# safijari/yag-slam

Measured on AMD Instinct MI355X. Metric: pose hypotheses/sec, higher is better.
Workload: dtype u8

## Files before the change

yag_slam_amd/csrc/ym_host_enqueue.hpp:

```cpp
void enqueue_prepare(ym_matcher *m, const CallPlan &P) {
    ym::PrepareArgs a;
    a.scans = P.d_scans; a.items = P.d_items; a.g = P.g; a.lat = P.lc; a.states = m->states.p; a.qlocal = m->qlocal.p;
    a.cells = m->cells.p; a.bbox = m->bbox.p; a.ctrig = m->ctrig.p; a.hypcell = m->hypcell.p; a.probs = P.probs;
    a.max_n = P.max_n; a.max_base = P.max_base; a.nt_stride = P.nt_stride; a.dim_stride = P.dim_stride; a.stamps = P.stamps;
    a.use_inline = P.inline_desc ? 1 : 0;
    a.pad0 = 0;
    std::memset(&a.inl, 0, sizeof a.inl);
    if (a.use_inline) {
        a.inl.item = P.hi[0];
        for (int i = 0; i < P.nscans; i++) a.inl.scans[i] = P.hs[i];
    }
    a.qnp = m->qnp.p; a.jobs = P.d_jobs; a.job_slot = P.d_job_slot;
    a.fault = nullptr; a.step = 0; a.pad1 = 0;
    for (int k = 0; k < 4; k++) a.cell_box[k] = P.cell_box[k];
    if (P.chain_step) { a.fault = m->seq_fault.p; a.step = P.chain_step; }
    a.tile_max_zero = P.use_tile_list ? m->tile_max.p : nullptr;
    const size_t lds = YM_PREP_LDS_BYTES(P.max_n);
    if (P.split_prepare) {
        if (P.n_jobs > 0) hipLaunchKernelGGL(ym::points_kernel, dim3(P.n_jobs), dim3(YM_POINTS_THREADS), lds, m->stream, a);
        hipLaunchKernelGGL(ym::cells_kernel, dim3(P.max_base + 1, P.B), dim3(256), 0, m->stream, a);
    } else {
        if (P.B == 1 && m->prepare_threads != 512)
            hipLaunchKernelGGL(ym::prepare_kernel<1024>, dim3(P.max_base + 2, P.B), dim3(1024), lds, m->stream, a);
        else
            hipLaunchKernelGGL(ym::prepare_kernel<512>, dim3(P.max_base + 2, P.B), dim3(512), lds, m->stream, a);
    }
}

int enqueue_select(ym_matcher *m, const CallPlan &P) {
    if (P.g.zone_count <= 1) return YM_OK;
    const size_t pts = (size_t)P.max_base * P.max_n;
    int log2cap = 10;
    while (((size_t)3 << log2cap) < 4 * pts) log2cap++;
    if (log2cap > 17 || P.g.storage_w >= 32768)
        return set_err(YM_ERR_UNSUPPORTED, "order-dependent smear (smear_deviation/resolution = %g): chains of more than 98304 readings are not supported",
                       m->cfg.smear_deviation / m->cfg.resolution);
    if (log2cap > 14 || m->select_global) {
        const size_t cap = (size_t)1 << log2cap;
        const int nb = 5;
        int rc = m->sel_scratch.ensure((size_t)P.B * cap * (3 + (nb - 1)));
        if (rc) return rc;
        ym::SelectGlobalArgs g;
        g.cells = m->cells.p; g.max_n = P.max_n; g.max_base = P.max_base; g.z2max = m->z2max; g.log2cap = log2cap;
        g.keys = m->sel_scratch.p; g.status = g.keys + (size_t)P.B * cap; g.minidx = g.status + (size_t)P.B * cap; g.nbr = g.minidx + (size_t)P.B * cap;
        HIP_TRY(hipMemsetAsync(g.keys, 0, (size_t)2 * P.B * cap * sizeof(unsigned), m->stream));
        HIP_TRY(hipMemsetAsync(g.minidx, 0xff, (size_t)P.B * cap * sizeof(unsigned), m->stream));
        const size_t lds = cap;
        hipLaunchKernelGGL(ym::select_global_kernel<5>, dim3(P.B), dim3(1024), lds, m->stream, g);
        return YM_OK;
    }
    if (m->z2max <= 1 && P.B <= m->select_split_max) {
        const size_t cap = (size_t)1 << log2cap;
        const size_t had = m->sel_tables.cap;
        int rc = m->sel_tables.ensure((size_t)2 * P.B * cap);
        if (rc) return rc;
        if (m->sel_tables.cap != had) HIP_TRY(hipMemsetAsync(m->sel_tables.p, 0, m->sel_tables.cap * sizeof(unsigned), m->stream));
        if ((rc = m->sel_rec.ensure((size_t)P.B * 12 * 1024))) return rc;
        if ((rc = m->sel_slot.ensure((size_t)P.B * pts))) return rc;
        ym::SelectSplitArgs s;
        s.cells = m->cells.p; s.max_n = P.max_n; s.max_base = P.max_base; s.log2cap = log2cap; s.pad = 0;
        s.keys = m->sel_tables.p; s.mx = s.keys + (size_t)P.B * cap; s.rec = m->sel_rec.p; s.slot_of = m->sel_slot.p; s.stamps = P.stamps;
        const dim3 grid((unsigned)((pts + YM_SELECT_SPLIT_THREADS - 1) / YM_SELECT_SPLIT_THREADS), P.B);
        hipLaunchKernelGGL(ym::select_hash_kernel, grid, dim3(YM_SELECT_SPLIT_THREADS), 0, m->stream, s);
        hipLaunchKernelGGL(ym::select_neighbours_kernel, grid, dim3(YM_SELECT_SPLIT_THREADS), 0, m->stream, s);
        hipLaunchKernelGGL(ym::select_relax_kernel, dim3(P.B), dim3(1024), cap, m->stream, s);
        return YM_OK;
    }
    ym::SelectArgs a;
    a.cells = m->cells.p; a.max_n = P.max_n; a.max_base = P.max_base; a.z2max = m->z2max; a.log2cap = log2cap; a.stamps = P.stamps;
    const size_t lds = (size_t)9 << log2cap;
    hipLaunchKernelGGL(ym::select_kernel<5>, dim3(P.B), dim3(1024), lds, m->stream, a);
    return YM_OK;
}

int enqueue_raster(ym_matcher *m, const CallPlan &P) {
    hipStream_t st = m->stream;
    const YmGeom &g = P.g;
    if (P.use_tile_list) {
        ym::TilesArgs t;
        t.bbox = m->bbox.p; t.tile_list = m->tile_list.p; t.tile_count = m->tile_count.p; t.tile_zero = m->tile_zero.p;
        t.tile_max = m->tile_max.p;
        t.hits = P.use_tile_hits ? m->tile_hits.p : nullptr; t.tile_h = P.tile_h;
        t.hit_limit = m->raster_hits_per_tile > 0 ? std::min(m->raster_hits_per_tile, YM_TILE_HITS) : YM_TILE_HITS;
        t.max_n = P.max_n; t.max_base = P.max_base; t.half_kernel = g.half_kernel;
        t.tiles_x = P.tiles_x; t.tiles_y = P.tiles_y; t.tile_cap = P.tile_cap;
        for (int k = 0; k < 4; k++) t.launch[k] = P.launch[k];
        hipLaunchKernelGGL(ym::tiles_kernel, dim3(P.B), dim3(YM_TILES_THREADS),
                           (size_t)4 * ((P.tiles_x * P.tiles_y + 31) / 32) + (P.use_tile_hits ? (size_t)8 * P.tile_cap : 0), st, t);
    }
    ym::RasterArgs a;
    a.tiles_x = P.tiles_x; a.tiles_y = P.tiles_y; a.tile_x0 = P.launch[0]; a.tile_y0 = P.launch[1]; a.ltx = P.ltx;
    a.tile_list = P.use_tile_list ? m->tile_list.p : nullptr; a.tile_count = m->tile_count.p; a.tile_cap = P.tile_cap;
    a.cells = m->cells.p; a.bbox = m->bbox.p; a.states = m->states.p; a.g = g; a.grid = m->grid.p;
    a.grid_stride = P.grid_stride; a.planes = m->planes.p; a.lut = m->ktab.p; a.max_n = P.max_n; a.max_base = P.max_base; a.stamps = P.stamps;
    a.tile_zero = m->tile_zero.p; a.sub_zero = m->sub_zero.p; a.planes_only = m->raster_planes_only;
    a.n_rowtab = m->raster_no_rowtab ? 0 : m->n_rowtab; a.rowtab = reinterpret_cast<const uint2 *>(m->rowtab.p); a.rowtab_shift = m->rowtab_shift; a.no_planes = P.win_only ? 1 : 0;
    const size_t rlds = YM_RASTER_LDS_BYTES(P.tile_h, g.half_kernel, a.n_rowtab);
    a.tile_max = m->tile_max.p; a.tile_max_host = P.use_tile_list ? reinterpret_cast<int32_t *>(m->tile_max_host.p) : nullptr;
    a.hits = (P.use_tile_list && P.use_tile_hits) ? m->tile_hits.p : nullptr; a.lty = P.lty; a.pad0 = 0;
    int rc;
    hipEvent_t ev_k = nullptr;
    if ((rc = prof_begin(m, 1, &ev_k))) return rc;
    if (P.ltx > 0 && P.lty > 0) {
        const int hint = m->tile_max_host.p ? *reinterpret_cast<volatile int32_t *>(m->tile_max_host.p) : 0;
        const int gx = m->raster_gx > 0 ? std::min(P.ltx * P.lty, m->raster_gx)
                                        : hint > 0 ? std::min(P.ltx * P.lty, hint + hint / 8 + 2) : P.ltx * P.lty;
        a.first_overflow = gx;
        if (P.use_tile_list) {
            if (P.tile_h == YM_TILE_H_TALL) {
                hipLaunchKernelGGL((ym::raster_kernel<128, false, YM_TILE_H_TALL, true>), dim3(gx, P.B), dim3(128), rlds, st, a);
                if (gx < P.ltx * P.lty) hipLaunchKernelGGL((ym::raster_kernel<128, true, YM_TILE_H_TALL, true>), dim3(4, P.B), dim3(128), rlds, st, a);
            } else {
                hipLaunchKernelGGL((ym::raster_kernel<128, false, YM_TILE_H, true>), dim3(gx, P.B), dim3(128), rlds, st, a);
                if (gx < P.ltx * P.lty) hipLaunchKernelGGL((ym::raster_kernel<128, true, YM_TILE_H, true>), dim3(4, P.B), dim3(128), rlds, st, a);
            }
        } else {
            if (P.tile_h == YM_TILE_H_TALL) hipLaunchKernelGGL((ym::raster_kernel<256, false, YM_TILE_H_TALL, false>), dim3(P.ltx * P.lty, P.B), dim3(256), rlds, st, a);
            else hipLaunchKernelGGL((ym::raster_kernel<256, false, YM_TILE_H, false>), dim3(P.ltx * P.lty, P.B), dim3(256), rlds, st, a);
        }
    }
    return prof_end(m, ev_k);
}

int enqueue_correlate(ym_matcher *m, const CallPlan &P);
void enqueue_score(ym_matcher *m, Slot &slot, const CallPlan &P);

int enqueue_yagpy_passes(ym_matcher *m, Slot &slot, const CallPlan &P) {
    const Call &call = slot.call;
    const YmGeom &g = P.g;
    m->sums_pass_offset[0] = 0;
    m->sums_pass_offset[1] = (size_t)P.B * P.yvol;
    for (int pass = 0; pass < (call.refine ? 2 : 1); pass++) {
        ym::YagArgs a;
        std::memset(&a, 0, sizeof a);
        a.g = g; a.pass = pass; a.penalize = call.penalize; a.refine = call.refine;
        a.last = (pass == 1 || !call.refine) ? 1 : 0;
        if (pass == 0) {
            a.search_xy = m->cfg.search_size * 0.5; a.step_xy = g.res * 2;
            a.search_t = m->cfg.coarse_search_angle_offset * 0.5; a.step_t = m->cfg.coarse_angle_resolution;
        } else {
            a.search_xy = g.res * 2; a.step_xy = g.res; a.search_t = 0.0349 * 0.5; a.step_t = 0.00349;
        }
        a.coarse_angle_res = m->cfg.coarse_angle_resolution;
        a.states = m->states.p; a.host_out = reinterpret_cast<YmItemState *>(slot.result.dp);
        a.qlocal = m->qlocal.p; a.axes = m->yaxes.p; a.rot = nullptr;
        a.sums = m->sums.p + m->sums_pass_offset[pass]; a.out = m->resp.p;
        a.grid = m->grid.p; a.grid_stride = P.grid_stride; a.vol_stride = P.yvol;
        a.max_n = P.max_n; a.maxd = P.ymaxd; a.maxt = P.ymaxt;
        hipLaunchKernelGGL(ym::yag_setup_kernel, dim3(1, P.B), dim3(256), 0, m->stream, a);
        if (pass == 0 && P.lc.nx > 0) {
            a.lat_nx = P.lc.nx; a.lat_ny = P.lc.ny; a.lat_nt = P.lc.nt; a.step_cells = P.sx;
            a.nt_stride = P.nt_stride; a.dim_stride = P.dim_stride; a.ctrig = m->ctrig.p; a.hypcell = m->hypcell.p;
            a.lsums = m->sums.p + (size_t)2 * P.B * P.yvol; a.lsums_stride = P.sums_c; a.counters = m->yag_counters.p;
            hipLaunchKernelGGL(ym::yag_lattice_kernel, dim3(P.B), dim3(256), 0, m->stream, a);
            int rc = enqueue_correlate(m, P);
            if (rc) return rc;
            enqueue_score(m, slot, P);
        }
        if (pass == 1 && m->yag_fast) {
            a.fine_rows = m->yag_fast;
            a.n_items = P.B;
            if (P.B >= 64) hipLaunchKernelGGL(ym::yag_fine_kernel<64>, dim3(8 * P.ymaxt * ((P.B + 7) / 8)), dim3(64), 0, m->stream, a);
            else hipLaunchKernelGGL(ym::yag_fine_kernel<256>, dim3(8 * P.ymaxt * ((P.B + 7) / 8)), dim3(256), 0, m->stream, a);
        }
        hipLaunchKernelGGL(ym::yag_score_kernel, dim3((P.ymaxd * P.ymaxd + 255) / 256, P.ymaxt, P.B), dim3(256), 0, m->stream, a);
        if (P.B >= 16) hipLaunchKernelGGL(ym::yag_reduce_kernel<256>, dim3(P.B), dim3(256), 0, m->stream, a);
        else hipLaunchKernelGGL(ym::yag_reduce_kernel<1024>, dim3(P.B), dim3(1024), 0, m->stream, a);
    }
    return YM_OK;
}

ym::RegionArgs region_args(ym_matcher *m, const CallPlan &P) {
    ym::RegionArgs r;
// ... 212 lines not shown
```

yag_slam_amd/csrc/ym_k_prepare.hpp:

```cpp
#pragma once

namespace ym {

#define YM_PREP_LDS_BYTES(max_n) ((size_t)(max_n) * 25 + ((size_t)(max_n) / 64 + 2) * 4 + 16)
#define YM_INLINE_SCANS 16
#ifndef YM_CELLS_Q
#define YM_CELLS_Q 3
#endif
struct YmInlineDesc {
    YmItem item;
    YmScanRef scans[YM_INLINE_SCANS];
};
struct PrepareArgs {
    const YmScanRef *scans;
    const YmItem *items;
    int32_t use_inline;
    int32_t pad0;
    YmInlineDesc inl;
    YmGeom g;
    YmLattice lat;
    YmItemState *states;
    double2 *qlocal;
    int32_t *qnp;
    YmCell *cells;
    int4 *bbox;
    double2 *ctrig;
    int32_t *hypcell;
    double *probs;
    int32_t max_n, max_base, nt_stride, dim_stride;
    const int32_t *jobs;
    const int32_t *job_slot;
    unsigned long long *stamps;
    int32_t *fault;
    int32_t step, pad1;
    int32_t cell_box[4];
    int32_t *tile_max_zero;
};

struct PrepLds {
    double *sx, *sy;
    int *nxt, *ex, *ent;
    unsigned char *chain;
};
__device__ __forceinline__ PrepLds prep_lds(unsigned char *raw, int max_n) {
    PrepLds l;
    l.sx = reinterpret_cast<double *>(raw);
    l.sy = l.sx + max_n;
    l.nxt = reinterpret_cast<int *>(l.sy + max_n);
    l.ex = l.nxt + max_n;
    l.ent = l.ex + max_n;
    l.chain = reinterpret_cast<unsigned char *>(l.ent + max_n / 64 + 2);
    return l;
}

template <int NT>
__device__ __forceinline__ int project_points(const YmScanRef &sr, double px, double py, double pt, bool yag, double *sx, double *sy,
                                              int *s_cnt , int32_t *cidx_out = nullptr) {
    constexpr int NW = NT / 64;
    const int tid = threadIdx.x;
    const int lane_ = tid & 63, wave_ = tid >> 6;
    const int per = (sr.n + NT - 1) / NT;
    auto valid = [&](int i, double &r) {
        r = 0.0;
        if (i >= sr.n) return false;
        r = sr.ranges[i];
        return yag ? !(r > sr.range_threshold || isnan(r)) : (r >= sr.min_range && r <= sr.range_threshold);
    };
    for (int k = 0; k < per; k++) {
        double r;
        const unsigned long long m = __ballot(valid(k * NT + tid, r));
        if (lane_ == 0) s_cnt[k * NW + wave_] = __popcll(m);
    }
    __syncthreads();
    int running = 0;
    for (int k = 0; k < per; k++) {
        const int i = k * NT + tid;
        double r;
        const bool ok = valid(i, r);
        const unsigned long long m = __ballot(ok);
        int before = 0, total = 0;
#pragma unroll
        for (int w = 0; w < NW; w++) {
            const int c = s_cnt[k * NW + w];
            before += w < wave_ ? c : 0;
            total += c;
        }
        const int pos = running + before + __popcll(m & ((1ull << lane_) - 1ull));
        if (ok) {
            const double angle = pt + sr.min_angle + i * sr.angle_inc;
            sx[pos] = px + r * cos(angle);
            sy[pos] = py + r * sin(angle);
        }
        if (cidx_out && i < sr.n) cidx_out[i] = ok ? pos : -1;
        running += total;
    }
    __syncthreads();
    return running;
}

template <int NT>
__device__ __forceinline__ int project_points_indexed(const YmScanRef &sr, double px, double py, double pt, const PrepLds &l, bool with_gov) {
    for (int i = threadIdx.x; i < sr.n; i += NT) {
        const int pos = sr.cidx[i];
        const double r = sr.ranges[i];
        if (pos >= 0) {
            const double angle = pt + sr.min_angle + i * sr.angle_inc;
            l.sx[pos] = px + r * cos(angle);
            l.sy[pos] = py + r * sin(angle);
        }
    }
    if (with_gov) {
        const int2 *gov = reinterpret_cast<const int2 *>(sr.gov);
        for (int i = threadIdx.x; i < sr.cnp; i += NT) {
            const int2 g = gov[i];
            l.nxt[i] = g.x;
            l.ex[i] = g.y;
        }
    }
    __syncthreads();
    return sr.cnp;
}

#define YM_CHAIN_GUARD 1e-9
#define YM_CHAIN_POSE_LIMIT 1.0e4
#define YM_CHAIN_HEADING_LIMIT 1.0e3
template <int NT, bool GUARD = false>
__device__ __forceinline__ int mark_chain(const PrepLds &l, int np, bool yag) {
    const int tid = threadIdx.x;
    const double min_sq = yag ? 0.2 * 0.2 : 0.1 * 0.1;
    int near = 0;
    for (int i = tid; i < np; i += NT) {
        const double fx = l.sx[i], fy = l.sy[i];
        int j = i + 1;
        for (; j < np; j++) {
            const double dx = fx - l.sx[j], dy = fy - l.sy[j];
            const double d2 = dx * dx + dy * dy;
            if (GUARD) near |= fabs(d2 - min_sq) <= YM_CHAIN_GUARD ? 1 : 0;
            if (d2 > min_sq) break;
        }
        l.nxt[i] = j;
        l.chain[i] = 0;
    }
    int unsafe = 0;
    if (GUARD) unsafe = __syncthreads_or(near);
    else __syncthreads();
    constexpr int SEG = 64;
    const int nseg = (np + SEG - 1) / SEG;
    for (int i = tid; i < np; i += NT) {
        const int seg_end = min(np, (i / SEG + 1) * SEG);
        int j = l.nxt[i];
        while (j < seg_end) j = l.nxt[j];
        l.ex[i] = j;
    }
    for (int i = tid; i < nseg; i += NT) l.ent[i] = -1;
    __syncthreads();
    if (tid == 0)
        for (int cur = 0; cur < np; cur = l.ex[cur]) l.ent[cur / SEG] = cur;
    __syncthreads();
    for (int sgi = tid; sgi < nseg; sgi += NT) {
        int c = l.ent[sgi];
        if (c >= 0) {
// ... 60 lines not shown
    if (tid < a.lat.nt) {
        const double angle = (sr.pose[2] - a.lat.angle_off) + tid * a.lat.angle_res;
        a.ctrig[(size_t)b * a.nt_stride + tid] = make_double2(cos(angle), sin(angle));
    }
    for (int i = tid; i < a.lat.nx * a.lat.ny; i += NT) a.probs[(size_t)b * a.lat.nx * a.lat.ny + i] = 0.0;
    int32_t *cx = a.hypcell + (size_t)b * 2 * a.dim_stride;
    int32_t *cy = cx + a.dim_stride;
    for (int i = tid; i < a.lat.nx; i += NT) cx[i] = hyp_cell(sr.pose[0], -a.lat.off_x, i, a.lat.step_x, off_x, a.g);
    for (int i = tid; i < a.lat.ny; i += NT) cy[i] = hyp_cell(sr.pose[1], -a.lat.off_y, i, a.lat.step_y, off_y, a.g);
    __syncthreads();
    {
        const int stx = kt_round_int(a.lat.step_x * a.g.scale), sty = kt_round_int(a.lat.step_y * a.g.scale);
        int ok = a.g.kpitch == 0;
        for (int i = tid; i < a.lat.nx; i += NT) ok &= (cx[i] == cx[0] + i * stx);
        for (int i = tid; i < a.lat.ny; i += NT) ok &= (cy[i] == cy[0] + i * sty);
        ok = __syncthreads_and(ok);
        if (tid == 0) a.states[b].regular[0] = ok;
    }
}

__device__ __forceinline__ void chain_check_cell(const PrepareArgs &a, int2 c) {
    if (a.fault && c.x != YM_CELL_NONE && (c.x < a.cell_box[0] || c.y < a.cell_box[1] || c.x > a.cell_box[2] || c.y > a.cell_box[3]))
        atomicCAS(a.fault, 0, a.step);
}

template <int NT, typename PT, typename GOV>
__device__ __forceinline__ void prepare_cells(const PrepareArgs &a, int b, int slot, int np, bool yag, double vpx, double vpy,
                                              double off_x, double off_y, PT pt_of, GOV gov_of) {
    const int tid = threadIdx.x;
    const int n_cchunks = YM_N_BOXES(a.max_n);
    YmCell *cells = a.cells + ((size_t)b * a.max_base + slot) * a.max_n;
    int4 *bbox = a.bbox + ((size_t)b * a.max_base + slot) * n_cchunks;
    for (int i0 = 0; i0 < n_cchunks * YM_BOX_CELLS; i0 += NT) {
        const int i = i0 + tid;
        int2 c = make_int2(YM_CELL_NONE, YM_CELL_NONE);
        if (i < np) {
            bool keep = false;
            const int2 g = gov_of(i);
            if (g.x >= 0 && g.y < np) {
                const double2 f = pt_of(g.x), cp = pt_of(g.y);
                const double fx = f.x, fy = f.y, cx = cp.x, cy = cp.y;
                const double aa = vpy - fy;
                const double bb = fx - vpx;
                const double cc = fy * vpx - fx * vpy;
                const double ss = cx * aa + cy * bb + cc;
                keep = yag ? (ss > 0.0) : !(ss < 0.0);
            }
            if (keep) {
                const double2 p = pt_of(i);
                int gx, gy;
                if (yag) {
                    gx = (int)rint((p.x - off_x) / a.g.res);
                    gy = (int)rint((p.y - off_y) / a.g.res);
                } else {
                    gx = world_to_grid(p.x, off_x, a.g.scale);
                    gy = world_to_grid(p.y, off_y, a.g.scale);
                }
                if (gx >= 0 && gx < a.g.roi_w && gy >= 0 && gy < a.g.roi_w)
                    c = make_int2(gx + a.g.border - a.g.win_origin, gy + a.g.border - a.g.win_origin);
            }
        }
        const bool has = c.x != YM_CELL_NONE;
        if (i < a.max_n) cells[i] = has ? ym_cell_pack(c.x, c.y) : ym_cell_none();
        chain_check_cell(a, c);
        const int x0 = row16_reduce(has ? c.x : INT32_MAX, OpMinI()), y0 = row16_reduce(has ? c.y : INT32_MAX, OpMinI());
        const int x1 = row16_reduce(has ? c.x : INT32_MIN, OpMaxI()), y1 = row16_reduce(has ? c.y : INT32_MIN, OpMaxI());
        if ((tid & (YM_BOX_CELLS - 1)) == 0 && i / YM_BOX_CELLS < n_cchunks) bbox[i / YM_BOX_CELLS] = make_int4(x0, y0, x1, y1);
    }
}

template <int NT>
__device__ __forceinline__ void clear_slot(const PrepareArgs &a, int b, int slot) {
    const int n_cchunks = YM_N_BOXES(a.max_n);
    YmCell *cells = a.cells + ((size_t)b * a.max_base + slot) * a.max_n;
    int4 *bbox = a.bbox + ((size_t)b * a.max_base + slot) * n_cchunks;
    for (int i = threadIdx.x; i < a.max_n; i += NT) cells[i] = ym_cell_none();
    for (int i = threadIdx.x; i < n_cchunks; i += NT) bbox[i] = make_int4(INT32_MAX, INT32_MAX, INT32_MIN, INT32_MIN);
}

template <int NT>
__device__ __forceinline__ void cells_from_cache(const PrepareArgs &a, int b, int slot, const YmScanRef &sr, const YmScanRef &qr, bool yag) {
    constexpr int Q = NT == 256 ? YM_CELLS_Q : 4;
    const double2 *__restrict__ cpts = reinterpret_cast<const double2 *>(sr.cache + YM_CACHE_HEADER);
    const YmGov *__restrict__ cgov = reinterpret_cast<const YmGov *>(sr.cache + YM_CACHE_HEADER + (size_t)sr.n * 16);
    const int np = *reinterpret_cast<const int *>(sr.cache);
    const double off_x = qr.pose[0] - (0.5 * (a.g.roi_w - 1) * a.g.res);
    const double off_y = qr.pose[1] - (0.5 * (a.g.roi_w - 1) * a.g.res);
    const double vpx = qr.pose[0], vpy = qr.pose[1];
    const int tid = threadIdx.x;
    const int n_cchunks = YM_N_BOXES(a.max_n);
    YmCell *cells = a.cells + ((size_t)b * a.max_base + slot) * a.max_n;
    int4 *bbox = a.bbox + ((size_t)b * a.max_base + slot) * n_cchunks;
    for (int i0 = 0; i0 < n_cchunks * YM_BOX_CELLS; i0 += Q * NT) {
        YmGov g[Q];
        YmCell cw[Q];
        double2 f[Q], t[Q];
        {
            double2 p[Q];
#pragma unroll
            for (int q = 0; q < Q; q++) {
                const int i = i0 + q * NT + tid;
                g[q] = i < np ? cgov[i] : ym_gov_pack(make_int2(-1, np));
                p[q] = cpts[i < np ? i : 0];
            }
#pragma unroll
            for (int q = 0; q < Q; q++) {
                int gx, gy;
                if (yag) {
                    gx = (int)rint((p[q].x - off_x) / a.g.res);
                    gy = (int)rint((p[q].y - off_y) / a.g.res);
                } else {
                    gx = world_to_grid(p[q].x, off_x, a.g.scale);
                    gy = world_to_grid(p[q].y, off_y, a.g.scale);
                }
                cw[q] = (gx >= 0 && gx < a.g.roi_w && gy >= 0 && gy < a.g.roi_w) ? ym_cell_pack(gx + a.g.border - a.g.win_origin, gy + a.g.border - a.g.win_origin)
                                                                                 : ym_cell_none();
            }
        }
        __builtin_amdgcn_sched_barrier(0);
#pragma unroll
        for (int q = 0; q < Q; q++) {
            const int2 st = ym_gov_unpack(g[q]);
            const bool decided = st.x >= 0 && st.y < np;
            f[q] = cpts[decided ? st.x : 0];
            t[q] = cpts[decided ? st.y : 0];
        }
#pragma unroll
        for (int q = 0; q < Q; q++) {
            const int i = i0 + q * NT + tid;
            if (i0 + q * NT >= n_cchunks * YM_BOX_CELLS) break;
            const int2 st = ym_gov_unpack(g[q]);
            bool keep = false;
            if (i < np && st.x >= 0 && st.y < np) {
                const double fx = f[q].x, fy = f[q].y, cx = t[q].x, cy = t[q].y;
                const double aa = vpy - fy;
                const double bb = fx - vpx;
                const double cc = fy * vpx - fx * vpy;
                const double ss = cx * aa + cy * bb + cc;
                keep = yag ? (ss > 0.0) : !(ss < 0.0);
            }
            const YmCell w = keep ? cw[q] : ym_cell_none();
            const int2 c = ym_cell_unpack(w);
            const bool has = c.x != YM_CELL_NONE;
            if (i < a.max_n) cells[i] = w;
            chain_check_cell(a, c);
            const int x0 = row16_reduce(has ? c.x : INT32_MAX, OpMinI()), y0 = row16_reduce(has ? c.y : INT32_MAX, OpMinI());
            const int x1 = row16_reduce(has ? c.x : INT32_MIN, OpMaxI()), y1 = row16_reduce(has ? c.y : INT32_MIN, OpMaxI());
            if ((tid & (YM_BOX_CELLS - 1)) == 0 && i / YM_BOX_CELLS < n_cchunks) bbox[i / YM_BOX_CELLS] = make_int4(x0, y0, x1, y1);
        }
    }
}

template <int NT>
__global__ __launch_bounds__(NT) void prepare_kernel(PrepareArgs a) {
    extern __shared__ __attribute__((aligned(16))) unsigned char lds_raw[];
    __shared__ int s_cnt[(YM_MAX_BEAMS / NT + 1) * (NT / 64)];
    if (a.stamps && threadIdx.x == 0 && blockIdx.x == 0 && blockIdx.y == 0) a.stamps[28] = wall_clock64() - a.stamps[19];
    YM_STAMP(a, 0);
    const int b = blockIdx.y;
    if (a.tile_max_zero && blockIdx.x == 0 && b == 0 && threadIdx.x == 0) *a.tile_max_zero = 0;
    const YmItem it = a.use_inline ? a.inl.item : a.items[b];
    const bool is_query = blockIdx.x == 0;
    const int slot = (int)blockIdx.x - 1;
    if ((int)blockIdx.x == a.max_base + 1) {
        YmScanRef qr = a.use_inline ? a.inl.scans[it.query] : a.scans[it.query];
        if (qr.pose_dev) { qr.pose[0] = qr.pose_dev[0]; qr.pose[1] = qr.pose_dev[1]; qr.pose[2] = qr.pose_dev[2]; }
        const double off_x = qr.pose[0] - (0.5 * (a.g.roi_w - 1) * a.g.res);
        const double off_y = qr.pose[1] - (0.5 * (a.g.roi_w - 1) * a.g.res);
        init_item<NT>(a, b, it, qr, -1, b, a.qlocal + (size_t)b * a.max_n, off_x, off_y);
        YM_STAMP_B1(a, 21);
        return;
    }
    if (!is_query && slot >= it.base_count) {
        clear_slot<NT>(a, b, slot);
        return;
    }
    const int si = is_query ? it.query : it.base_begin + slot;
    YmScanRef sr = a.use_inline ? a.inl.scans[si] : a.scans[si];
    YmScanRef qr = a.use_inline ? a.inl.scans[it.query] : a.scans[it.query];
    if (sr.pose_dev) { sr.pose[0] = sr.pose_dev[0]; sr.pose[1] = sr.pose_dev[1]; sr.pose[2] = sr.pose_dev[2]; }
    if (qr.pose_dev) { qr.pose[0] = qr.pose_dev[0]; qr.pose[1] = qr.pose_dev[1]; qr.pose[2] = qr.pose_dev[2]; }
    if (a.fault && *a.fault) {
        if (!is_query) { clear_slot<NT>(a, b, slot); return; }
        sr.n = 0;
    }
    const bool yag = a.g.semantics == 1;
    if (!is_query && sr.cache && !sr.stale) {
        cells_from_cache<NT>(a, b, slot, sr, qr, yag);
        return;
    }
    const PrepLds l = prep_lds(lds_raw, a.max_n);
    const double px = (is_query && yag) ? 0.0 : sr.pose[0];
    const double py = (is_query && yag) ? 0.0 : sr.pose[1];
    const double pt = (is_query && yag) ? 0.0 : sr.pose[2];
    const bool indexed = sr.cidx != nullptr && sr.n > 0;
    const int np = indexed ? project_points_indexed<NT>(sr, px, py, pt, l, !is_query) : project_points<NT>(sr, px, py, pt, yag, l.sx, l.sy, s_cnt);
    YM_STAMP(a, 1);
    YM_STAMP_B1(a, 20);
    const double off_x = qr.pose[0] - (0.5 * (a.g.roi_w - 1) * a.g.res);
    const double off_y = qr.pose[1] - (0.5 * (a.g.roi_w - 1) * a.g.res);
    if (is_query) {
        store_query_local<NT>(sr, l, np, yag, a.qlocal + (size_t)b * a.max_n);
        if (threadIdx.x == 0) { a.qnp[b] = np; a.states[b].nq = np; }
        YM_STAMP(a, 2);
        YM_STAMP(a, 18);
        return;
    }
    const int2 *known = reinterpret_cast<const int2 *>(sr.gov);
    if (!known) mark_chain<NT>(l, np, yag);
    YM_STAMP_B1(a, 22);
    if (sr.cache) store_cache<NT>(sr, l, np, yag);
    if (indexed)
        prepare_cells<NT>(a, b, slot, np, yag, qr.pose[0], qr.pose[1], off_x, off_y,
                          [&](int i) { return make_double2(l.sx[i], l.sy[i]); }, [&](int i) { return make_int2(l.nxt[i], l.ex[i]); });
    else if (known)
        prepare_cells<NT>(a, b, slot, np, yag, qr.pose[0], qr.pose[1], off_x, off_y,
                          [&](int i) { return make_double2(l.sx[i], l.sy[i]); }, [&](int i) { return known[i]; });
    else
        prepare_cells<NT>(a, b, slot, np, yag, qr.pose[0], qr.pose[1], off_x, off_y,
                          [&](int i) { return make_double2(l.sx[i], l.sy[i]); }, [&](int i) { return gov_walk(l, i, np, yag); });
    YM_STAMP_B1(a, 23);
}

struct StructureArgs {
    YmScanRef sr;
    int32_t *gov[2];
    int32_t *cidx[2];
    int32_t *info;
    double *ranges_out;
    uint32_t *done;
    uint32_t serial;
    uint32_t pad;
};
template <int NT>
__device__ __forceinline__ void structure_body(const StructureArgs &a, int sem, unsigned char *lds_raw, int *s_cnt) {
    const bool yag = sem == 1;
    const PrepLds l = prep_lds(lds_raw, a.sr.n);
    const int np = project_points<NT>(a.sr, 0.0, 0.0, 0.0, yag, l.sx, l.sy, s_cnt, yag ? a.cidx[1] : a.cidx[0]);
    const int unsafe = mark_chain<NT, true>(l, np, yag);
    int2 *gov = reinterpret_cast<int2 *>(yag ? a.gov[1] : a.gov[0]);
    for (int i = threadIdx.x; i < np; i += NT) gov[i] = gov_walk(l, i, np, yag);
    if (a.ranges_out && sem == 0)
        for (int i = threadIdx.x; i < a.sr.n; i += NT) a.ranges_out[i] = a.sr.ranges[i];
    if (threadIdx.x == 0) { a.info[2 * sem] = np; a.info[2 * sem + 1] = unsafe; }
    if (a.done) {
        __syncthreads();
        if (threadIdx.x == 0) {
            __threadfence_system();
            __hip_atomic_store(a.done + sem, a.serial, __ATOMIC_RELEASE, __HIP_MEMORY_SCOPE_SYSTEM);
        }
    }
}
template <int NT>
__global__ __launch_bounds__(NT) void structure_kernel(StructureArgs a) {
    extern __shared__ __attribute__((aligned(16))) unsigned char lds_raw[];
    __shared__ int s_cnt[(YM_MAX_BEAMS / NT + 1) * (NT / 64)];
    structure_body<NT>(a, (int)blockIdx.x, lds_raw, s_cnt);
}
template <int NT>
__global__ __launch_bounds__(NT) void structure_many_kernel(const StructureArgs *table) {
    extern __shared__ __attribute__((aligned(16))) unsigned char lds_raw[];
    __shared__ int s_cnt[(YM_MAX_BEAMS / NT + 1) * (NT / 64)];
    const StructureArgs a = table[blockIdx.y];
    structure_body<NT>(a, (int)blockIdx.x, lds_raw, s_cnt);
}

#define YM_POINTS_THREADS 256
__global__ __launch_bounds__(YM_POINTS_THREADS) void points_kernel(PrepareArgs a) {
    constexpr int NT = YM_POINTS_THREADS;
    extern __shared__ __attribute__((aligned(16))) unsigned char lds_raw[];
    __shared__ int s_cnt[(YM_MAX_BEAMS / NT + 1) * (NT / 64)];
    const int job = a.jobs[blockIdx.x];
    const bool is_query = job < 0;
    const YmScanRef sr = a.scans[job & 0x7fffffff];
    const bool yag = a.g.semantics == 1;
    const PrepLds l = prep_lds(lds_raw, a.max_n);
    const double px = (is_query && yag) ? 0.0 : sr.pose[0];
    const double py = (is_query && yag) ? 0.0 : sr.pose[1];
    const double pt = (is_query && yag) ? 0.0 : sr.pose[2];
    const int np = (sr.cidx && sr.n > 0) ? project_points_indexed<NT>(sr, px, py, pt, l, false)
                                         : project_points<NT>(sr, px, py, pt, yag, l.sx, l.sy, s_cnt);
    if (is_query) {
        const int qs = a.job_slot[blockIdx.x];
        store_query_local<NT>(sr, l, np, yag, sr.qcache ? reinterpret_cast<double2 *>(sr.qcache + YM_CACHE_HEADER) : a.qlocal + (size_t)qs * a.max_n);
        if (threadIdx.x == 0) *(sr.qcache ? reinterpret_cast<int *>(sr.qcache) : a.qnp + qs) = np;
        return;
    }
    if (!sr.gov) mark_chain<NT>(l, np, yag);
    store_cache<NT>(sr, l, np, yag);
}

__global__ __launch_bounds__(256) void cells_kernel(PrepareArgs a) {
    constexpr int NT = 256;
    const int b = blockIdx.y;
    if (a.tile_max_zero && blockIdx.x == 0 && b == 0 && threadIdx.x == 0) *a.tile_max_zero = 0;
    const YmItem it = a.items[b];
    const int slot = (int)blockIdx.x - 1;
    const YmScanRef qr = a.scans[it.query];
    if (blockIdx.x == 0) {
        const int qs = it.pad;
        const double off_x = qr.pose[0] - (0.5 * (a.g.roi_w - 1) * a.g.res);
        const double off_y = qr.pose[1] - (0.5 * (a.g.roi_w - 1) * a.g.res);
        const double2 *ql = qr.qcache ? reinterpret_cast<const double2 *>(qr.qcache + YM_CACHE_HEADER) : a.qlocal + (size_t)qs * a.max_n;
        init_item<NT>(a, b, it, qr, qr.qcache ? *reinterpret_cast<const int *>(qr.qcache) : a.qnp[qs], qs, ql, off_x, off_y);
        return;
    }
    if (slot >= it.base_count) {
        clear_slot<NT>(a, b, slot);
        return;
    }
    cells_from_cache<NT>(a, b, slot, a.scans[it.base_begin + slot], qr, a.g.semantics == 1);
}

#define YM_TILES_THREADS 256
struct TilesArgs {
    const int4 *bbox;
    uint32_t *tile_list;
    int32_t *tile_count;
    int32_t *tile_max;
    const uint8_t *tile_zero;
    int32_t max_n, max_base, half_kernel;
    int32_t tiles_x, tiles_y, tile_cap;
    int32_t launch[4];
    uint16_t *hits;
    int32_t tile_h;
    int32_t hit_limit;
};
__global__ __launch_bounds__(YM_TILES_THREADS) void tiles_kernel(TilesArgs a) {
    extern __shared__ unsigned tile_bits[];
    __shared__ int s_n;
    constexpr int NT = YM_TILES_THREADS;
    const int tid = threadIdx.x, b = blockIdx.x;
    const int ntiles = a.tiles_x * a.tiles_y, nwords = (ntiles + 31) / 32;
    const int h = a.half_kernel;
    const int lx0 = a.launch[0], ly0 = a.launch[1], lx1 = a.launch[2], ly1 = a.launch[3];
    const int ltx = lx1 - lx0 + 1, lty = ly1 - ly0 + 1, nsub = ltx * lty;
    int *cnt = reinterpret_cast<int *>(tile_bits + nwords);
    int *fill = cnt + nsub;
    for (int i = tid; i < nwords; i += NT) tile_bits[i] = 0u;
    if (a.hits)
        for (int i = tid; i < nsub; i += NT) cnt[i] = 0;
    if (tid == 0) s_n = 0;
    __syncthreads();
    const int n_boxes = a.max_base * YM_N_BOXES(a.max_n);
    const int4 *bbox = a.bbox + (size_t)b * n_boxes;
    const int th_shift = a.tile_h == YM_TILE_H_TALL ? 6 : 5;
    static_assert(YM_TILE_H == 32 && YM_TILE_H_TALL == 64, "tile heights as shifts");
    for (int c = tid; c < n_boxes; c += NT) {
        const int4 bb = bbox[c];
        if (bb.x > bb.z) continue;
        const int tx0 = max(lx0, max(bb.x - h, 0) / YM_TILE_W), tx1 = min(lx1, (bb.z + h) / YM_TILE_W);
        const int ty0 = max(ly0, max(bb.y - h, 0) >> th_shift), ty1 = min(ly1, (bb.w + h) >> th_shift);
        for (int ty = ty0; ty <= ty1; ty++)
            for (int tx = tx0; tx <= tx1; tx++) {
                const int t = ty * a.tiles_x + tx;
                atomicOr(&tile_bits[t >> 5], 1u << (t & 31));
                if (a.hits) atomicAdd(&cnt[(ty - ly0) * ltx + (tx - lx0)], 1);
            }
    }
    __syncthreads();
    const uint8_t *tz = a.tile_zero + (size_t)b * ntiles;
    uint32_t *list = a.tile_list + (size_t)b * a.tile_cap;
    for (int i = tid; i < nsub; i += NT) {
        const int ty = ly0 + i / ltx, tx = lx0 + i % ltx, t = ty * a.tiles_x + tx;
        const bool hit = (tile_bits[t >> 5] >> (t & 31)) & 1u;
        if (hit || tz[t] == 0) {
            const int at = atomicAdd(&s_n, 1);
            const uint32_t nh = !a.hits ? 0xffffu : cnt[i] > a.hit_limit ? 0xffffu : (uint32_t)cnt[i];
            list[at] = (uint32_t)(t | (hit ? 0 : 0x8000)) | nh << 16;
            if (a.hits) fill[i] = at << 16;
        }
    }
    __syncthreads();
    if (tid == 0) {
        a.tile_count[b] = s_n;
        if (s_n > *reinterpret_cast<volatile int32_t *>(a.tile_max)) atomicMax(a.tile_max, s_n);
    }
    if (!a.hits) return;
    uint16_t *hits = a.hits + (size_t)b * a.tile_cap * YM_TILE_HITS;
    const int n_cchunks = YM_N_BOXES(a.max_n);
    for (int c = tid; c < n_boxes; c += NT) {
        const int4 bb = bbox[c];
        if (bb.x > bb.z) continue;
        const int slot = c / n_cchunks;
        const uint16_t first_cell = (uint16_t)(slot * a.max_n + (c - slot * n_cchunks) * YM_BOX_CELLS);
        const int tx0 = max(lx0, max(bb.x - h, 0) / YM_TILE_W), tx1 = min(lx1, (bb.z + h) / YM_TILE_W);
        const int ty0 = max(ly0, max(bb.y - h, 0) >> th_shift), ty1 = min(ly1, (bb.w + h) >> th_shift);
        for (int ty = ty0; ty <= ty1; ty++)
            for (int tx = tx0; tx <= tx1; tx++) {
                const int i = (ty - ly0) * ltx + (tx - lx0);
                if (cnt[i] > a.hit_limit) continue;
                const int old = atomicAdd(&fill[i], 1);
                hits[(size_t)(old >> 16) * YM_TILE_HITS + (old & 0xffff)] = first_cell;
            }
    }
}

struct SelectArgs {
    YmCell *cells;
    int32_t max_n, max_base;
    int32_t z2max;
    int32_t log2cap;
    unsigned long long *stamps;
};

__device__ __forceinline__ unsigned select_key(int x, int y) {
    return ((unsigned)(y + 32768) << 16) | ((unsigned)(x + 32768) & 0xffffu);
}
__device__ __forceinline__ int select_find(const unsigned *keys, unsigned bmask, int shift, unsigned key) {
    unsigned bk = (key * 2654435761u) >> shift;
    for (;;) {
        const uint4 q = *reinterpret_cast<const uint4 *>(keys + 4 * bk);
        if (q.x == key) return (int)(4 * bk);
        if (q.y == key) return (int)(4 * bk + 1);
        if (q.z == key) return (int)(4 * bk + 2);
        if (q.w == key) return (int)(4 * bk + 3);
        if (q.w == 0u) return -1;
        bk = (bk + 1u) & bmask;
    }
}
__device__ __forceinline__ int select_find_from(const unsigned *keys, unsigned bmask, unsigned bk, unsigned key) {
    for (;;) {
        const uint4 q = *reinterpret_cast<const uint4 *>(keys + 4 * bk);
        if (q.x == key) return (int)(4 * bk);
        if (q.y == key) return (int)(4 * bk + 1);
        if (q.z == key) return (int)(4 * bk + 2);
        if (q.w == key) return (int)(4 * bk + 3);
        if (q.w == 0u) return -1;
        bk = (bk + 1u) & bmask;
    }
}
__device__ __forceinline__ int select_insert(unsigned *keys, unsigned bmask, int shift, unsigned key) {
    unsigned bk = (key * 2654435761u) >> shift;
    for (;;) {
        const uint4 q = *reinterpret_cast<const uint4 *>(keys + 4 * bk);
        int j = (q.x == key || q.x == 0u) ? 0 : (q.y == key || q.y == 0u) ? 1 : (q.z == key || q.z == 0u) ? 2 : (q.w == key || q.w == 0u) ? 3 : 4;
        for (; j < 4; j++) {
            const unsigned prev = atomicCAS(&keys[4 * bk + j], 0u, key);
            if (prev == 0u || prev == key) return (int)(4 * bk + j);
        }
        bk = (bk + 1u) & bmask;
    }
}

template <int NB>
__global__ __launch_bounds__(1024) void select_kernel(SelectArgs a) {
    constexpr int NT = 1024, NW = (NB - 1) / 4;
    constexpr int PMAX = 12;
    constexpr int DX[9] = {0, 1, -1, 0, 0, 1, 1, -1, -1};
    constexpr int DY[9] = {0, 0, 0, 1, -1, 1, -1, 1, -1};
    extern __shared__ unsigned sel_lds[];
    const int b = blockIdx.x, tid = threadIdx.x;
    const unsigned cap = 1u << a.log2cap, bmask = (cap >> 2) - 1u;
    const int shift = 32 - (a.log2cap - 2);
    unsigned *keys = sel_lds;
    unsigned *minidx = sel_lds + cap;
    unsigned char *status = reinterpret_cast<unsigned char *>(sel_lds + 2 * cap);
    YM_STAMP(a, 24);
    YmCell *cells = a.cells + (size_t)b * a.max_base * a.max_n;
    const int total = a.max_base * a.max_n;
    int2 mine[PMAX];
    unsigned short slot_of[PMAX];
    const int per = (total + NT - 1) / NT, e0 = tid * per;
#pragma unroll
    for (int q = 0; q < PMAX; q++) {
        const int e = e0 + q;
        mine[q] = (q < per && e < total) ? ym_cell_unpack(cells[e]) : make_int2(YM_CELL_NONE, YM_CELL_NONE);
    }
    for (unsigned i = tid; i < cap; i += NT) { keys[i] = 0u; minidx[i] = 0xffffffffu; status[i] = 0; }
    __syncthreads();
    YM_STAMP(a, 25);
#pragma unroll
    for (int q = 0; q < PMAX; q++) {
        slot_of[q] = 0;
        if (mine[q].x == YM_CELL_NONE) continue;
        const int slot = select_insert(keys, bmask, shift, select_key(mine[q].x, mine[q].y));
        slot_of[q] = (unsigned short)slot;
        atomicMin(&minidx[slot], (unsigned)(e0 + q));
    }
    __syncthreads();
    YM_STAMP(a, 26);
    unsigned long long nb[PMAX][NW];
    unsigned und = 0;
#pragma unroll
    for (int k = 0; k < PMAX; k++) {
#pragma unroll
        for (int w = 0; w < NW; w++) nb[k][w] = ~0ull;
        if (mine[k].x == YM_CELL_NONE) continue;
        const unsigned s = slot_of[k], me = (unsigned)(e0 + k);
        if (minidx[s] != me) continue;
        const int x = mine[k].x, y = mine[k].y;
        bool any = false;
        unsigned nkey[NB], nbk[NB];
        uint4 nq[NB];
#pragma unroll
        for (int n = 1; n < NB; n++) {
            nkey[n] = select_key(x + DX[n], y + DY[n]);
            nbk[n] = (nkey[n] * 2654435761u) >> shift;
            nq[n] = *reinterpret_cast<const uint4 *>(keys + 4 * nbk[n]);
        }
#pragma unroll
        for (int n = 1; n < NB; n++) {
            const uint4 q4 = nq[n];
            const unsigned key = nkey[n];
            int t = q4.x == key ? (int)(4 * nbk[n]) : q4.y == key ? (int)(4 * nbk[n] + 1) : q4.z == key ? (int)(4 * nbk[n] + 2)
                    : q4.w == key ? (int)(4 * nbk[n] + 3) : q4.w == 0u ? -1 : -2;
            if (t == -2) t = select_find_from(keys, bmask, (nbk[n] + 1u) & bmask, key);
            if (t >= 0 && minidx[t] < me) {
                any = true;
                const int j = n - 1;
                nb[k][j >> 2] &= ~(0xffffull << (16 * (j & 3)));
                nb[k][j >> 2] |= (unsigned long long)(unsigned)t << (16 * (j & 3));
            }
        }
        if (any) und |= 1u << k;
        else status[s] = 1;
    }
    YM_STAMP(a, 3);
    unsigned char *vst = status;
    unsigned wmask = 0;
#pragma unroll
    for (int k = 0; k < PMAX; k++) wmask |= __ballot((und >> k) & 1u) ? (1u << k) : 0u;
    while (wmask) {
        unsigned m = wmask;
        while (m) {
            const int k = __builtin_ctz(m);
            m &= m - 1;
            bool still = false;
            asm volatile("" ::: "memory");
            if ((und >> k) & 1u) {
                bool knocked = false, pending = false;
#pragma unroll
                for (int j = 0; j < NB - 1; j++) {
                    const unsigned t = (unsigned)(nb[k][j >> 2] >> (16 * (j & 3))) & 0xffffu;
                    if (t != 0xffffu) {
                        const unsigned char stt = vst[t];
                        knocked |= stt == 1;
                        pending |= stt == 0;
                    }
                }
                const unsigned s = slot_of[k];
                if (knocked) vst[s] = 2;
                else if (!pending) vst[s] = 1;
                else still = true;
                if (!still) und &= ~(1u << k);
            }
            if (__ballot(still) == 0ull) wmask &= ~(1u << k);
        }
// ... 242 lines not shown
```

Measured before the change: 13.86 billion.

## Stage cached points in LDS for cells kernel and prefetch boxes in tiles kernel

```diff
diff --git a/yag_slam_amd/csrc/ym_host_enqueue.hpp b/yag_slam_amd/csrc/ym_host_enqueue.hpp
--- a/yag_slam_amd/csrc/ym_host_enqueue.hpp
+++ b/yag_slam_amd/csrc/ym_host_enqueue.hpp
@@ -18,7 +18,10 @@
     const size_t lds = YM_PREP_LDS_BYTES(P.max_n);
     if (P.split_prepare) {
         if (P.n_jobs > 0) hipLaunchKernelGGL(ym::points_kernel, dim3(P.n_jobs), dim3(YM_POINTS_THREADS), lds, m->stream, a);
-        hipLaunchKernelGGL(ym::cells_kernel, dim3(P.max_base + 1, P.B), dim3(256), 0, m->stream, a);
+        if (P.max_n <= YM_CELLS_STAGED_MAX_N)
+            hipLaunchKernelGGL(ym::cells_kernel<true>, dim3(P.max_base + 1, P.B), dim3(256), YM_CELLS_STAGED_LDS_BYTES(P.max_n), m->stream, a);
+        else
+            hipLaunchKernelGGL(ym::cells_kernel<false>, dim3(P.max_base + 1, P.B), dim3(256), 0, m->stream, a);
     } else {
         if (P.B == 1 && m->prepare_threads != 512)
             hipLaunchKernelGGL(ym::prepare_kernel<1024>, dim3(P.max_base + 2, P.B), dim3(1024), lds, m->stream, a);
diff --git a/yag_slam_amd/csrc/ym_k_prepare.hpp b/yag_slam_amd/csrc/ym_k_prepare.hpp
--- a/yag_slam_amd/csrc/ym_k_prepare.hpp
+++ b/yag_slam_amd/csrc/ym_k_prepare.hpp
@@ -7,6 +7,9 @@
 #ifndef YM_CELLS_Q
 #define YM_CELLS_Q 3
 #endif
+#define YM_CELLS_GROUP 5
+#define YM_CELLS_STAGED_MAX_N 1440
+#define YM_CELLS_STAGED_LDS_BYTES(max_n) ((size_t)(max_n) * 16)
 struct YmInlineDesc {
     YmItem item;
     YmScanRef scans[YM_INLINE_SCANS];
@@ -373,6 +376,94 @@
 }
 
 template <int NT>
+__device__ __forceinline__ void cells_from_cache_staged(const PrepareArgs &a, int b, int slot, const YmScanRef &sr, const YmScanRef &qr, bool yag,
+                                                        double2 *lp ) {
+    constexpr int G = YM_CELLS_GROUP;
+    typedef const __attribute__((address_space(1))) double *global_f64;
+    typedef const __attribute__((address_space(1))) YmGov *global_gov;
+    const global_f64 cpts = (global_f64)reinterpret_cast<const double *>(sr.cache + YM_CACHE_HEADER);
+    const global_gov cgov = (global_gov)reinterpret_cast<const YmGov *>(sr.cache + YM_CACHE_HEADER + (size_t)sr.n * 16);
+    auto point = [&](int i) { return make_double2(cpts[2 * (size_t)i], cpts[2 * (size_t)i + 1]); };
+    const int np = *reinterpret_cast<const int *>(sr.cache);
+    const double off_x = qr.pose[0] - (0.5 * (a.g.roi_w - 1) * a.g.res);
+    const double off_y = qr.pose[1] - (0.5 * (a.g.roi_w - 1) * a.g.res);
+    const double vpx = qr.pose[0], vpy = qr.pose[1];
+    const int tid = threadIdx.x;
+    const int n_cchunks = YM_N_BOXES(a.max_n);
+    const int n_pad = n_cchunks * YM_BOX_CELLS;
+    YmCell *cells = a.cells + ((size_t)b * a.max_base + slot) * a.max_n;
+    int4 *bbox = a.bbox + ((size_t)b * a.max_base + slot) * n_cchunks;
+    auto cell_of = [&](const double2 &p) {
+        int gx, gy;
+        if (yag) {
+            gx = (int)rint((p.x - off_x) / a.g.res);
+            gy = (int)rint((p.y - off_y) / a.g.res);
+        } else {
+            gx = world_to_grid(p.x, off_x, a.g.scale);
+            gy = world_to_grid(p.y, off_y, a.g.scale);
+        }
+        return (gx >= 0 && gx < a.g.roi_w && gy >= 0 && gy < a.g.roi_w) ? ym_cell_pack(gx + a.g.border - a.g.win_origin, gy + a.g.border - a.g.win_origin)
+                                                                         : ym_cell_none();
+    };
+    YmGov g[G];
+    YmCell cw[G];
+    {
+        double2 p[G];
+#pragma unroll
+        for (int q = 0; q < G; q++) {
+            const int i = q * NT + tid;
+            g[q] = i < np ? cgov[i] : ym_gov_pack(make_int2(-1, np));
+            p[q] = point(i < np ? i : 0);
+        }
+#pragma unroll
+        for (int q = 0; q < G; q++) {
+            const int i = q * NT + tid;
+            if (i < np) lp[i] = p[q];
+            cw[q] = cell_of(p[q]);
+        }
+    }
+    for (int i = G * NT + tid; i < np; i += NT) lp[i] = point(i);
+    __syncthreads();
+    auto finish = [&](int i, YmGov gv, YmCell cell) {
+        const int2 st = ym_gov_unpack(gv);
+        bool keep = false;
+        if (i < np && st.x >= 0 && st.y < np) {
+            const double2 f = lp[st.x], t = lp[st.y];
+            const double fx = f.x, fy = f.y, cx = t.x, cy = t.y;
+            const double aa = vpy - fy;
+            const double bb = fx - vpx;
+            const double cc = fy * vpx - fx * vpy;
+            const double ss = cx * aa + cy * bb + cc;
+            keep = yag ? (ss > 0.0) : !(ss < 0.0);
+        }
+        const YmCell w = keep ? cell : ym_cell_none();
+        const int2 c = ym_cell_unpack(w);
+        const bool has = c.x != YM_CELL_NONE;
+        if (i < a.max_n) cells[i] = w;
+        chain_check_cell(a, c);
+        const int x0 = row16_reduce(has ? c.x : INT32_MAX, OpMinI()), y0 = row16_reduce(has ? c.y : INT32_MAX, OpMinI());
+        const int x1 = row16_reduce(has ? c.x : INT32_MIN, OpMaxI()), y1 = row16_reduce(has ? c.y : INT32_MIN, OpMaxI());
+        if ((tid & (YM_BOX_CELLS - 1)) == 0 && i / YM_BOX_CELLS < n_cchunks) bbox[i / YM_BOX_CELLS] = make_int4(x0, y0, x1, y1);
+    };
+#pragma unroll
+    for (int q = 0; q < G; q++)
+        if (q * NT < n_pad) finish(q * NT + tid, g[q], cw[q]);
+    for (int i0 = G * NT; i0 < n_pad; i0 += G * NT) {
+        YmGov g2[G];
+#pragma unroll
+        for (int q = 0; q < G; q++) {
+            const int i = i0 + q * NT + tid;
+            g2[q] = i < np ? cgov[i] : ym_gov_pack(make_int2(-1, np));
+        }
+#pragma unroll
+        for (int q = 0; q < G; q++) {
+            const int i = i0 + q * NT + tid;
+            if (i0 + q * NT < n_pad) finish(i, g2[q], i < np ? cell_of(lp[i]) : ym_cell_none());
+        }
+    }
+}
+
+template <int NT>
 __global__ __launch_bounds__(NT) void prepare_kernel(PrepareArgs a) {
     extern __shared__ __attribute__((aligned(16))) unsigned char lds_raw[];
     __shared__ int s_cnt[(YM_MAX_BEAMS / NT + 1) * (NT / 64)];
@@ -511,7 +602,9 @@
     store_cache<NT>(sr, l, np, yag);
 }
 
+template <bool STAGED>
 __global__ __launch_bounds__(256) void cells_kernel(PrepareArgs a) {
+    extern __shared__ __attribute__((aligned(16))) unsigned char lds_raw[];
     constexpr int NT = 256;
     const int b = blockIdx.y;
     if (a.tile_max_zero && blockIdx.x == 0 && b == 0 && threadIdx.x == 0) *a.tile_max_zero = 0;
@@ -530,10 +623,13 @@
         clear_slot<NT>(a, b, slot);
         return;
     }
-    cells_from_cache<NT>(a, b, slot, a.scans[it.base_begin + slot], qr, a.g.semantics == 1);
+    if (STAGED) cells_from_cache_staged<NT>(a, b, slot, a.scans[it.base_begin + slot], qr, a.g.semantics == 1, reinterpret_cast<double2 *>(lds_raw));
+    else cells_from_cache<NT>(a, b, slot, a.scans[it.base_begin + slot], qr, a.g.semantics == 1);
 }
 
 #define YM_TILES_THREADS 256
+#define YM_TILES_KEEP 3
+#define YM_TILES_KEEP_Z 2
 struct TilesArgs {
     const int4 *bbox;
     uint32_t *tile_list;
@@ -558,18 +654,30 @@
     const int ltx = lx1 - lx0 + 1, lty = ly1 - ly0 + 1, nsub = ltx * lty;
     int *cnt = reinterpret_cast<int *>(tile_bits + nwords);
     int *fill = cnt + nsub;
+    const int n_boxes = a.max_base * YM_N_BOXES(a.max_n);
+    const int4 *bbox = a.bbox + (size_t)b * n_boxes;
+    const uint8_t *tz = a.tile_zero + (size_t)b * ntiles;
+    int4 mine[YM_TILES_KEEP];
+    uint8_t zero_of[YM_TILES_KEEP_Z];
+#pragma unroll
+    for (int k = 0; k < YM_TILES_KEEP; k++) {
+        const int c = k * NT + tid;
+        mine[k] = c < n_boxes ? bbox[c] : make_int4(INT32_MAX, INT32_MAX, INT32_MIN, INT32_MIN);
+    }
+#pragma unroll
+    for (int k = 0; k < YM_TILES_KEEP_Z; k++) {
+        const int i = k * NT + tid;
+        zero_of[k] = i < nsub ? tz[(ly0 + i / ltx) * a.tiles_x + lx0 + i % ltx] : (uint8_t)1;
+    }
     for (int i = tid; i < nwords; i += NT) tile_bits[i] = 0u;
     if (a.hits)
         for (int i = tid; i < nsub; i += NT) cnt[i] = 0;
     if (tid == 0) s_n = 0;
     __syncthreads();
-    const int n_boxes = a.max_base * YM_N_BOXES(a.max_n);
-    const int4 *bbox = a.bbox + (size_t)b * n_boxes;
     const int th_shift = a.tile_h == YM_TILE_H_TALL ? 6 : 5;
     static_assert(YM_TILE_H == 32 && YM_TILE_H_TALL == 64, "tile heights as shifts");
-    for (int c = tid; c < n_boxes; c += NT) {
-        const int4 bb = bbox[c];
-        if (bb.x > bb.z) continue;
+    auto mark = [&](const int4 &bb) {
+        if (bb.x > bb.z) return;
         const int tx0 = max(lx0, max(bb.x - h, 0) / YM_TILE_W), tx1 = min(lx1, (bb.z + h) / YM_TILE_W);
         const int ty0 = max(ly0, max(bb.y - h, 0) >> th_shift), ty1 = min(ly1, (bb.w + h) >> th_shift);
         for (int ty = ty0; ty <= ty1; ty++)
@@ -578,20 +686,26 @@
                 atomicOr(&tile_bits[t >> 5], 1u << (t & 31));
                 if (a.hits) atomicAdd(&cnt[(ty - ly0) * ltx + (tx - lx0)], 1);
             }
-    }
-    __syncthreads();
-    const uint8_t *tz = a.tile_zero + (size_t)b * ntiles;
+    };
+#pragma unroll
+    for (int k = 0; k < YM_TILES_KEEP; k++) mark(mine[k]);
+    for (int c = YM_TILES_KEEP * NT + tid; c < n_boxes; c += NT) mark(bbox[c]);
+    __syncthreads();
     uint32_t *list = a.tile_list + (size_t)b * a.tile_cap;
-    for (int i = tid; i < nsub; i += NT) {
+    auto enlist = [&](int i, bool zero) {
         const int ty = ly0 + i / ltx, tx = lx0 + i % ltx, t = ty * a.tiles_x + tx;
         const bool hit = (tile_bits[t >> 5] >> (t & 31)) & 1u;
-        if (hit || tz[t] == 0) {
+        if (hit || !zero) {
             const int at = atomicAdd(&s_n, 1);
             const uint32_t nh = !a.hits ? 0xffffu : cnt[i] > a.hit_limit ? 0xffffu : (uint32_t)cnt[i];
             list[at] = (uint32_t)(t | (hit ? 0 : 0x8000)) | nh << 16;
             if (a.hits) fill[i] = at << 16;
         }
-    }
+    };
+#pragma unroll
+    for (int k = 0; k < YM_TILES_KEEP_Z; k++)
+        if (k * NT + tid < nsub) enlist(k * NT + tid, zero_of[k] != 0);
+    for (int i = YM_TILES_KEEP_Z * NT + tid; i < nsub; i += NT) enlist(i, tz[(ly0 + i / ltx) * a.tiles_x + lx0 + i % ltx] != 0);
     __syncthreads();
     if (tid == 0) {
         a.tile_count[b] = s_n;
@@ -600,9 +714,8 @@
     if (!a.hits) return;
     uint16_t *hits = a.hits + (size_t)b * a.tile_cap * YM_TILE_HITS;
     const int n_cchunks = YM_N_BOXES(a.max_n);
-    for (int c = tid; c < n_boxes; c += NT) {
-        const int4 bb = bbox[c];
-        if (bb.x > bb.z) continue;
+    auto scatter = [&](int c, const int4 &bb) {
+        if (bb.x > bb.z) return;
         const int slot = c / n_cchunks;
         const uint16_t first_cell = (uint16_t)(slot * a.max_n + (c - slot * n_cchunks) * YM_BOX_CELLS);
         const int tx0 = max(lx0, max(bb.x - h, 0) / YM_TILE_W), tx1 = min(lx1, (bb.z + h) / YM_TILE_W);
@@ -614,7 +727,10 @@
                 const int old = atomicAdd(&fill[i], 1);
                 hits[(size_t)(old >> 16) * YM_TILE_HITS + (old & 0xffff)] = first_cell;
             }
-    }
+    };
+#pragma unroll
+    for (int k = 0; k < YM_TILES_KEEP; k++) scatter(k * NT + tid, mine[k]);
+    for (int c = YM_TILES_KEEP * NT + tid; c < n_boxes; c += NT) scatter(c, bbox[c]);
 }
 
 struct SelectArgs {
```

Result: faster. 14.04 billion (median of 6 runs) (+1.3%).
